# YunjiKim/Unsupervised-Keypoint-Learning-for-Guiding-Class-conditional-Video-Prediction

Measured on AMD Instinct MI355X. Metric: detector_translator train frames/sec @128x128 K=15, higher is better.
Workload: dtype f32

## Files before the change

unsupervised-keypoint-learning-for-guiding-class-conditional-video-prediction_amd/csrc/conv_wgrad.hip:

```cpp
#include "kpx_internal.h"
#include "kpx_bf16.h"
#include <cassert>

#ifdef __HIP_DEVICE_COMPILE__
__device__ __attribute__((aligned(16))) float kpx_zero16[4] = {0.f, 0.f, 0.f, 0.f};
#else
extern __device__ float kpx_zero16[4];
#endif


template <int BMc, int BNk, int WM, int WN, bool VEC, bool MERGE>
__global__ __launch_bounds__(WM * WN * 64) void conv_wgrad_kernel(const WgradGeom g) {
    constexpr int NT = WM * WN * 64;
    constexpr int BKP = 32;
    constexpr int TM = BMc / (WM * 32), TN = BNk / (WN * 32);
    constexpr int RA = (BKP * BMc / 4) / NT, RB = (BKP * BNk / 4) / NT;
    static_assert(RA >= 1 && RB >= 1 && TM >= 1 && TN >= 1, "tile/wave shape");
    __shared__ __attribute__((aligned(16))) float As[2][BKP * BMc];
    __shared__ __attribute__((aligned(16))) float Bs[2][BKP * BNk];

    const int t = threadIdx.x, lane = t & 63, wave = t >> 6;
    const int li = lane & 31, lh = lane >> 5;
    const int wm = wave / WN, wn = wave % WN;
    int L = kpx_xcd_remap(blockIdx.x, gridDim.x);
// ... 511 lines not shown
            const float* p = g.x + ((ptrdiff_t)(n * g.Hi + ih) * g.Wi + iw0) * g.Cin + xf[i];
            const float v = *(ok ? p : g.x);
            rx[i] = ok ? v : 0.f;
        }
        {
            const int k4 = t % (CoutT / 4), px = t / (CoutT / 4), k = k4 * 4;
            my = 0;
            if (k < g.Cout) { const int rem = g.Cout - k; my = rem >= 4 ? 15u : (15u >> (4 - rem)); }
            const float* p = g.dy + ((size_t)(n * g.Ho + ho) * g.Wo + wc * CW + px) * g.lddy + k;
            ry = *reinterpret_cast<const f32x4*>(my ? p : g.dy);
        }
    };
    auto store_chunk = [&](int buf) {
#pragma unroll
        for (int i = 0; i < RX; ++i) xs[buf][t + 256 * i] = rx[i];
        f32x4 o;
#pragma unroll
        for (int j = 0; j < 4; ++j) o[j] = (my >> j) & 1u ? ry[j] : 0.f;
        *reinterpret_cast<f32x4*>(&dys[buf][t * 4]) = o;
    };
    const int nch = cend > cbeg ? cend - cbeg : 0;
    if (nch > 0) { load_chunk(cbeg); store_chunk(0); }
    __syncthreads();
    for (int ch = 0; ch < nch; ++ch) {
        const int buf = ch & 1;
        const bool more = ch + 1 < nch;
        if (more) load_chunk(cbeg + ch + 1);
#pragma unroll
        for (int sl = 0; sl < 2; ++sl) {
            const int r = wave + 4 * sl;
            if (r < g.KH) {
                const float* Xr = &xs[buf][r * SEG];
#pragma unroll
                for (int s2 = 0; s2 < CW / 2; ++s2) {
                    const int kp = 2 * s2 + lh;
                    acc[sl] = __builtin_amdgcn_mfma_f32_32x32x2f32(Xr[kp * g.Cin + li], dys[buf][kp * CoutT + li], acc[sl], 0, 0, 0);
                }
            }
        }
        if (more) store_chunk(buf ^ 1);
        __syncthreads();
    }
    float* out = g.out + (size_t)split * g.slab;
#pragma unroll
    for (int sl = 0; sl < 2; ++sl) {
        const int r = wave + 4 * sl;
        if (r < g.KH) {
#pragma unroll
            for (int e = 0; e < 16; ++e) {
                const int c = (e & 3) + 8 * (e >> 2) + 4 * lh;
                if (c < KWC && li < g.Cout) out[((size_t)r * KWC + c) * g.Cout + li] = acc[sl][e];
            }
        }
    }
}

static bool wgrad_rows_merged_plan(int N, int Ho, int Wo, int Cin, int Cout, int KH, int KW, int* S, int* cpb) {
    if (Cin % 4 == 0 || KW * Cin > 32 || (32 + KW - 1) * Cin > 128 || KH > 8 || KW < 2 || Wo % 32 != 0 || Cout > 32 ||
        (long)N * Ho * Wo < 65536)
        return false;
    const long total = (long)N * Ho * (Wo / 32);
    long s = total < 768 ? total : 768;
    *cpb = (int)((total + s - 1) / s);
    *S = (int)((total + *cpb - 1) / *cpb);
    return true;
}

static bool wgrad_rows_plan(int N, int Ho, int Wo, int Cin, int Cout, int KH, int KW, int* S, int* cpb, int* CT) {
    if (KH > 3 || KW > 3 || KH * KW < 2 || Wo % 32 != 0 || Cout > 32 || Cin > 128 || (long)N * Ho * Wo < 65536) return false;
    *CT = Cin > 32 ? 2 : 1;
    const int ct = (Cin + 32 * *CT - 1) / (32 * *CT);
    const long total = (long)N * Ho * (Wo / 32);
    long want = 768 / ct;
    if (want < 1) want = 1;
    long s = total < want ? total : want;
    const size_t slab_bytes = (size_t)KH * KW * Cin * Cout * 4;
    const size_t cap = (size_t)256 << 20;
    if ((size_t)s * slab_bytes > cap) s = (long)(cap / slab_bytes);
    if (s < 1) s = 1;
    *cpb = (int)((total + s - 1) / s);
    *S = (int)((total + *cpb - 1) / *cpb);
    return true;
}

static void wgrad_tiles(int Cin, int Cout, int& bm, int& bn) {
    auto pick = [](int c) { return ((c + 127) / 128 * 128 == (c + 63) / 64 * 64) ? 128 : 64; };
    bm = pick(Cin); bn = pick(Cout);
    if (bm != bn) { bm = 64; bn = 64; }
}

static inline bool wgrad_merge(int Cin, int ldx, int KW) { return Cin % 4 != 0 && ldx == Cin && KW > 1 && KW * Cin <= 64; }

static int wgrad_splits(int N, int Ho, int Wo, int Cin, int Cout, int KH, int KW) {
    int bm, bn;
    wgrad_tiles(Cin, Cout, bm, bn);
    long tiles = (long)KH * KW * ((Cin + bm - 1) / bm) * ((Cout + bn - 1) / bn);
    if (wgrad_merge(Cin, Cin, KW)) tiles = (long)KH * ((Cout + bn - 1) / bn);
    const long P = (long)N * Ho * Wo;
    const long target = bm == 128 ? 2560 : 4096;
    long S = target / tiles;
    const long maxS_pix = P / 512 > 0 ? P / 512 : 1;
    if (S > maxS_pix) S = maxS_pix;
    const size_t slab_bytes = (size_t)KH * KW * Cin * Cout * 4;
    const size_t cap = (size_t)256 << 20;
    if ((size_t)S * slab_bytes > cap) S = (long)(cap / slab_bytes);
    if (S < 1) S = 1;
    return (int)S;
}

enum { WG_F32, WG_BF16, WG_IMAGE16 };
struct WgradCall : WgradGeom { int arith, types; };

struct WgradPlan {
    int family = -1;
    int S; size_t need;
    int cpb, CT, bm;
    WgradGeom g;
};

static bool wgrad_args_ok(const WgradCall& c) {
    if (!c.x || !c.dy || c.N <= 0 || c.Hi <= 0 || c.Wi <= 0 || c.Cin <= 0 || c.Cout <= 0 || c.Ho <= 0 || c.Wo <= 0 || c.KH <= 0 || c.KW <= 0 ||
        c.stride <= 0 || c.ldx < c.Cin || c.lddy < c.Cout || c.arith < 0 || c.arith > 1)
        return false;
    if (c.types == WG_BF16) return c.ldx % 8 == 0 && c.lddy % 8 == 0 && kpx_aligned16(c.x, c.dy);
    return c.types != WG_IMAGE16 || c.Cin <= 4;
}

template <class G>
static G wgrad_fill(const WgradPlan& p) {
    const WgradGeom& c = p.g;
    G g{};
    g.x = c.x; g.dy = c.dy; g.out = c.out;
    g.N = c.N; g.Hi = c.Hi; g.Wi = c.Wi; g.Cin = c.Cin; g.ldx = c.ldx;
    g.Ho = c.Ho; g.Wo = c.Wo; g.Cout = c.Cout; g.lddy = c.lddy;
    g.KH = c.KH; g.KW = c.KW; g.pad_t = c.pad_t; g.pad_l = c.pad_l;
    g.total_chunks = c.N * c.Ho * (c.Wo / 32); g.cpb = p.cpb; g.ct = c.ct; g.slab = c.slab;
    return g;
}

static WgradPlan wgrad_plan(const WgradCall& c) {
    WgradPlan p{};
    WgradGeom& g = p.g = c;
    g.slab = (size_t)c.KH * c.KW * c.Cin * c.Cout;
    const bool any = !c.x;
    auto take = [&](int family, int S) {
        p.family = family; p.S = S;
        if (S > 1 && (size_t)S * g.slab * 4 > p.need) p.need = (size_t)S * g.slab * 4;
        return !any;
    };
    g.vecA = any || (c.ldx % 4 == 0 && kpx_aligned16(c.x)); g.vecB = any || (c.lddy % 4 == 0 && kpx_aligned16(c.dy));
    const bool vec = g.vecA && g.vecB;
    const size_t px_in = (size_t)c.N * c.Hi * c.Wi, px_out = (size_t)c.N * c.Ho * c.Wo;
    int S, bn;

    if (c.types != WG_BF16 && kpx_offsets_fit(px_in, c.ldx, 0x60000000ull) && kpx_offsets_fit(px_out, c.lddy, 0x60000000ull) &&
        (any || (c.Cout % 4 == 0 && g.vecB)) && (c.Cin % 4 != 0 || g.vecA)) {
        S = kpx_wsmall_splits(c.N, c.Hi, c.Wi, c.Cin, c.Ho, c.Wo, c.Cout, c.KH, c.KW, c.stride);
        if (S >= 1 && take(KPX_WGRAD_WSMALL, S)) return p;
    }
    if (c.types == WG_IMAGE16) return p;
    if (c.types == WG_F32 && c.stride == 1) {
        if (c.KH == 3 && c.KW == 3 && c.pad_t == 1 && c.pad_l == 1 && c.Ho == c.Hi && c.Wo == c.Wi && vec && (any || c.ldx >= ((c.Cin + 3) & ~3)) &&
            kpx_offsets_fit(px_in, c.ldx > c.lddy ? c.ldx : c.lddy, 0x60000000ull)) {
            S = kpx_wino_wgrad_splits(c.N, c.Hi, c.Wi, c.Cin, c.Cout);
            if (S >= 1 && take(KPX_WGRAD_WINO, S)) return p;
        }
        g.ct = 1;
        if (c.ldx == c.Cin && g.vecB && wgrad_rows_merged_plan(c.N, c.Ho, c.Wo, c.Cin, c.Cout, c.KH, c.KW, &S, &p.cpb) && take(KPX_WGRAD_ROWS_MERGED, S))
            return p;
        if (vec && c.Cin % 4 == 0 && wgrad_rows_plan(c.N, c.Ho, c.Wo, c.Cin, c.Cout, c.KH, c.KW, &S, &p.cpb, &p.CT)) {
            g.ct = (c.Cin + 32 * p.CT - 1) / (32 * p.CT);
            if (take(KPX_WGRAD_ROWS, S)) return p;
        }
    }
    wgrad_tiles(c.Cin, c.Cout, p.bm, bn);
    g.ct = (c.Cin + p.bm - 1) / p.bm; g.kt = (c.Cout + bn - 1) / bn; g.P = (int)px_out;
    g.S = S = wgrad_splits(c.N, c.Ho, c.Wo, c.Cin, c.Cout, c.KH, c.KW);
    g.pps = ((g.P + S - 1) / S + 31) / 32 * 32;
    g.io16 = c.types == WG_BF16;
    g.terms = g.io16 || c.arith == KPX_ARITH_BF16 ? 1 : 3;
    const bool tap = c.types == WG_F32 && vec && c.Cin % 4 == 0 && c.Cout % 4 == 0 && c.Wo % 32 == 0;
    if (kpx_wgrad3_eligible(&g) && (c.stride > 1 || !tap) && take(KPX_WGRAD_GEMM3, S)) return p;
    if (c.types == WG_BF16) return p;
    if (tap) {
        const int chunks = c.N * c.Ho * (c.Wo / 32);
        p.cpb = (chunks + S - 1) / S;
        const int St = (chunks + p.cpb - 1) / p.cpb;
        assert(St <= S);
        if (take(KPX_WGRAD_TAP_ROWS, St)) return p;
    }
    if (wgrad_merge(c.Cin, c.ldx, c.KW)) {
        g.merge = c.Cin; g.Cin = c.KW * c.Cin; g.KW = 1; g.vecA = 0;
        g.ct = (g.Cin + p.bm - 1) / p.bm;
    }
    take(KPX_WGRAD_GENERIC, S);
    return p;
}

static int wgrad_run(const WgradCall& c, float* dw, void* workspace, size_t workspace_bytes, void* stream) {
    if (!dw || !wgrad_args_ok(c)) return KPX_EINVAL;
    WgradPlan p = wgrad_plan(c);
    if (p.family < 0 || p.need > (workspace ? workspace_bytes : 0)) return KPX_EINVAL;
    float* const out = p.g.out = p.S > 1 ? (float*)workspace : dw;
    hipStream_t s = kpx_stream(stream);
    int rc = 0;
    switch (p.family) {
        case KPX_WGRAD_WSMALL:
            rc = kpx_wsmall_launch(c.x, c.N, c.Hi, c.Wi, c.Cin, c.ldx, c.dy, c.Ho, c.Wo, c.Cout, c.lddy, c.KH, c.KW, c.stride, c.pad_t, c.pad_l, out, p.S, s,
                                   c.types == WG_IMAGE16);
            break;
        case KPX_WGRAD_WINO:
            rc = kpx_wino_wgrad3x3(c.x, c.N, c.Hi, c.Wi, c.Cin, c.ldx, c.dy, c.Cout, c.lddy, out, p.S, s);
            break;
        case KPX_WGRAD_ROWS_MERGED:
        case KPX_WGRAD_ROWS: {
            const WgradRowsGeom r = wgrad_fill<WgradRowsGeom>(p);
            const dim3 grid((unsigned)(p.S * r.ct));
            if (p.family == KPX_WGRAD_ROWS_MERGED) hipLaunchKernelGGL((conv_wgrad_rows_merged_kernel<0>), grid, dim3(256), 0, s, r);
            else if (p.CT == 2) hipLaunchKernelGGL((conv_wgrad_rows_kernel<2>), grid, dim3(256), 0, s, r);
            else hipLaunchKernelGGL((conv_wgrad_rows_kernel<1>), grid, dim3(256), 0, s, r);
            break;
        }
        case KPX_WGRAD_TAP_ROWS: {
            WgradTapGeom r = wgrad_fill<WgradTapGeom>(p);
            r.stride = c.stride; r.S = p.S; r.kt = p.g.kt;
            const dim3 grid((unsigned)(r.S * r.KH * r.KW * r.ct * r.kt));
            if (p.bm == 128) hipLaunchKernelGGL((conv_wgrad_tap_rows_kernel<128, 128, 2, 4>), grid, dim3(512), 0, s, r);
            else hipLaunchKernelGGL((conv_wgrad_tap_rows_kernel<64, 64, 2, 2>), grid, dim3(256), 0, s, r);
            break;
        }
        default: {
            const WgradGeom& g = p.g;
            const dim3 grid((unsigned)(g.S * g.KH * g.KW * g.ct * g.kt));
            const bool vec = g.vecA && g.vecB;
            if (p.family == KPX_WGRAD_GEMM3) rc = kpx_wgrad3_launch(g, p.bm, g.terms, s);
            else if (g.merge) hipLaunchKernelGGL((conv_wgrad_kernel<64, 64, 2, 2, false, true>), grid, dim3(256), 0, s, g);
            else if (p.bm == 128 && vec) hipLaunchKernelGGL((conv_wgrad_kernel<128, 128, 2, 4, true, false>), grid, dim3(512), 0, s, g);
            else if (p.bm == 128) hipLaunchKernelGGL((conv_wgrad_kernel<128, 128, 2, 4, false, false>), grid, dim3(512), 0, s, g);
            else if (vec) hipLaunchKernelGGL((conv_wgrad_kernel<64, 64, 2, 2, true, false>), grid, dim3(256), 0, s, g);
            else hipLaunchKernelGGL((conv_wgrad_kernel<64, 64, 2, 2, false, false>), grid, dim3(256), 0, s, g);
        }
    }
    return finish_wgrad(rc ? rc : kpx_launch_status(), workspace, dw, p.g.slab, p.S, s);
}

extern "C" int kpx_conv2d_wgrad_f32(const float* x, int N, int Hi, int Wi, int Cin, int ldx,
                                    const float* dy, int Ho, int Wo, int Cout, int lddy,
                                    float* dw, int KH, int KW, int stride, int pad_t, int pad_l, int arith,
                                    void* workspace, size_t workspace_bytes, void* stream) {
    return wgrad_run({{x, dy, nullptr, N, Hi, Wi, Cin, ldx, Ho, Wo, Cout, lddy, KH, KW, stride, pad_t, pad_l}, arith, WG_F32}, dw, workspace, workspace_bytes, stream);
}

extern "C" int kpx_conv2d_wgrad_bf16(const void* x, int N, int Hi, int Wi, int Cin, int ldx, const void* dy, int Ho, int Wo, int Cout, int lddy,
                                     float* dw, int KH, int KW, int stride, int pad_t, int pad_l, void* workspace, size_t workspace_bytes, void* stream) {
    return wgrad_run({{(const float*)x, (const float*)dy, nullptr, N, Hi, Wi, Cin, ldx, Ho, Wo, Cout, lddy, KH, KW, stride, pad_t, pad_l}, 0, WG_BF16},
                     dw, workspace, workspace_bytes, stream);
}

extern "C" int kpx_conv_image_wgrad_bf16(const float* x, int N, int Hi, int Wi, int Cin, int ldx, const void* dy, int Ho, int Wo, int Cout, int lddy,
                                         float* dw, int KH, int KW, int stride, int pad_t, int pad_l, void* workspace, size_t workspace_bytes, void* stream) {
    return wgrad_run({{x, (const float*)dy, nullptr, N, Hi, Wi, Cin, ldx, Ho, Wo, Cout, lddy, KH, KW, stride, pad_t, pad_l}, 0, WG_IMAGE16},
                     dw, workspace, workspace_bytes, stream);
}

extern "C" int kpx_conv2d_wgrad_plan(const float* x, int N, int Hi, int Wi, int Cin, int ldx, const float* dy, int Ho, int Wo, int Cout, int lddy,
                                     int KH, int KW, int stride, int pad_t, int pad_l, int arith, int* family, int* splits, size_t* workspace_bytes) {
    const WgradCall c{{x, dy, nullptr, N, Hi, Wi, Cin, ldx, Ho, Wo, Cout, lddy, KH, KW, stride, pad_t, pad_l}, arith, WG_F32};
    if (!family || !splits || !workspace_bytes || !wgrad_args_ok(c)) return KPX_EINVAL;
    const WgradPlan p = wgrad_plan(c);
    *family = p.family; *splits = p.S; *workspace_bytes = p.need;
    return 0;
}

extern "C" size_t kpx_conv2d_wgrad_workspace_bytes(int N, int Ho, int Wo, int Cin, int Cout, int KH, int KW) {
    auto need = [&](int st) { return wgrad_plan({{nullptr, nullptr, nullptr, N, Ho * st, Wo * st, Cin, Cin, Ho, Wo, Cout, Cout, KH, KW, st, 1, 1}, 0, WG_F32}).need; };
    return std::max(need(1), need(2));
}
```

unsupervised-keypoint-learning-for-guiding-class-conditional-video-prediction_amd/csrc/conv_wino.hip:

```cpp
#include "kpx_internal.h"
#include "kpx_env.h"
#include <stdlib.h>
#include <type_traits>
#include <atomic>

struct WinoGeom {
    const float* x; float* y; const float* U; const float* bias;
    int N, H, W, Cin, ldx, Cout, ldy, act;
    int pack;
    int Kp, Np;
    int tiles_y, tiles_x, nt;
    int stagger;
    float* stats;
    const float* mask_y; int ld_mask;
    const float* bn_beta;
};

static __device__ __attribute__((aligned(16))) float wino_zero16[4] = {0.f, 0.f, 0.f, 0.f};

template <bool DGRAD>
__global__ __launch_bounds__(256) void wino_filter_transform_frag_kernel(const float* __restrict__ w, int Cin, int Cout, int Kp, int Np, float* __restrict__ Uf) {
    const int K = DGRAD ? Cout : Cin, Nn = DGRAD ? Cin : Cout;
    const int KC = Kp >> 3, NB = Np >> 5;
    const size_t total = (size_t)Kp * Np;
// ... 296 lines not shown
    }
    if (STATS != 0) {
        __syncthreads();
        float* const S = smem;
        *reinterpret_cast<f32x4*>(&S[t * 8]) = st_s;
        *reinterpret_cast<f32x4*>(&S[t * 8 + 4]) = st_q;
        __syncthreads();
        if (t < 2 * NC) {
            const int stat = t / NC, c = t - stat * NC, cq = c >> 2, e = c & 3;
            float r = 0.f;
#pragma unroll 8
            for (int m = 0; m < 512 / (NC / 4); ++m) r += S[(cq + (NC / 4) * m) * 8 + stat * 4 + e];
            const size_t tile_id = ((size_t)n * g.tiles_y + by) * g.tiles_x + bx;
            if (n0 + c < g.Cout) g.stats[(tile_id * 2 + stat) * g.Cout + n0 + c] = r;
        }
    }
#ifdef KPX_WINO_STAMP
    if (dbg) { dbg[3] = __builtin_amdgcn_s_memtime(); dbg[4] = __builtin_amdgcn_s_memrealtime(); }
#endif
}

static inline int w2_lds_bytes(int mode) { const int main = W2_MAIN * 4, epi = 4 * 2 * 64 * 32 * mode * 4; return main > epi ? main : epi; }

static std::atomic<unsigned long long> wino_attr_mask{0};

extern "C" int kpx_conv3x3_wino_eligible(int N, int H, int W, int K, int Nn, int ldin, const void* in_ptr) {
    if (kpx_env()->no_wino || N <= 0 || K <= 0 || Nn <= 0) return 0;
    const bool shape = (H % 16 == 0 && W % 16 == 0) || (H == 8 && W == 8 && N % 4 == 0);
    const int kmin = 4, nmin = 4;
    const bool kfit = ldin >= ((K + 7) & ~7) || K == 4;
    return shape && K >= kmin && Nn >= nmin && (K >= 16 || K == 4 || K == 8) && kfit && (ldin % 4 == 0) && (((uintptr_t)in_ptr) & 15) == 0;
}
extern "C" __attribute__((visibility("hidden"))) int kpx_wino_eligible(int N, int H, int W, int K, int Nn, int ldin, const void* in_ptr) {
    return kpx_conv3x3_wino_eligible(N, H, W, K, Nn, ldin, in_ptr);
}

extern "C" size_t kpx_wino_u_bytes(int Cin, int Cout) {
    const size_t a = (size_t)((Cin + 7) & ~7) * ((Cout + 31) & ~31), b = (size_t)((Cout + 7) & ~7) * ((Cin + 31) & ~31);
    return 16 * 4 * (a > b ? a : b);
}

extern "C" int kpx_wino_filter_transform_f32(const float* w_hwio, int Cin, int Cout, int dgrad, float* U, void* stream) {
    if (!w_hwio || !U || Cin <= 0 || Cout <= 0) return KPX_EINVAL;
    const int K = dgrad ? Cout : Cin, Nn = dgrad ? Cin : Cout;
    const int Kp = (K + 7) & ~7, Np = (Nn + 31) & ~31;
    const size_t pairs = (size_t)Kp * Np;
    size_t nb = (pairs + 255) / 256; if (nb > 1024) nb = 1024;
    hipStream_t s = kpx_stream(stream);
    if (dgrad) hipLaunchKernelGGL(wino_filter_transform_frag_kernel<true>, dim3((unsigned)nb), dim3(256), 0, s, w_hwio, Cin, Cout, Kp, Np, U);
    else hipLaunchKernelGGL(wino_filter_transform_frag_kernel<false>, dim3((unsigned)nb), dim3(256), 0, s, w_hwio, Cin, Cout, Kp, Np, U);
    return kpx_launch_status();
}

__global__ __launch_bounds__(256) void wino_filter_transform_batch_kernel(const KpxWinoDesc* __restrict__ descs) {
    const KpxWinoDesc d = descs[blockIdx.y];
    const int Cin = d.cin, Cout = d.cout;
    const bool dg = d.dgrad != 0;
    const int K = dg ? Cout : Cin, Nn = dg ? Cin : Cout;
    const int Kp = (K + 7) & ~7, Np = (Nn + 31) & ~31, KC = Kp >> 3, NB = Np >> 5;
    const size_t total = (size_t)Kp * Np, pstride = (size_t)KC * NB * 256;
    const float* __restrict__ w = d.w;
    float* __restrict__ Uf = d.u;
    for (size_t idx = (size_t)blockIdx.x * 256 + threadIdx.x; idx < total; idx += (size_t)gridDim.x * 256) {
        const int j = (int)(idx & 3), li = (int)((idx >> 2) & 31), lh = (int)((idx >> 7) & 1);
        const size_t blk = idx >> 8;
        const int nb = (int)(blk % NB), kc = (int)(blk / NB);
        const int c = 8 * kc + 4 * lh + j, n = 32 * nb + li;
        const bool real = c < K && n < Nn;
        float g[3][3];
#pragma unroll
        for (int r = 0; r < 3; ++r)
#pragma unroll
            for (int q = 0; q < 3; ++q)
                g[r][q] = !real ? 0.f : (dg ? w[((size_t)((2 - r) * 3 + (2 - q)) * Cin + n) * Cout + c] : w[((size_t)(r * 3 + q) * Cin + c) * Cout + n]);
        float t[4][3];
#pragma unroll
        for (int q = 0; q < 3; ++q) {
            t[0][q] = g[0][q];
            t[1][q] = 0.5f * (g[0][q] + g[1][q] + g[2][q]);
            t[2][q] = 0.5f * (g[0][q] - g[1][q] + g[2][q]);
            t[3][q] = g[2][q];
        }
        float* o = Uf + blk * 256 + (idx & 255);
#pragma unroll
        for (int i = 0; i < 4; ++i) {
            o[(size_t)(i * 4 + 0) * pstride] = t[i][0];
            o[(size_t)(i * 4 + 1) * pstride] = 0.5f * (t[i][0] + t[i][1] + t[i][2]);
            o[(size_t)(i * 4 + 2) * pstride] = 0.5f * (t[i][0] - t[i][1] + t[i][2]);
            o[(size_t)(i * 4 + 3) * pstride] = t[i][2];
        }
    }
}
extern "C" int kpx_wino_filter_transform_batch_f32(const void* descs_dev, int n, void* stream) {
    if (!descs_dev || n <= 0 || n > 65535) return KPX_EINVAL;
    hipLaunchKernelGGL(wino_filter_transform_batch_kernel, dim3(64, (unsigned)n), dim3(256), 0, kpx_stream(stream), (const KpxWinoDesc*)descs_dev);
    return kpx_launch_status();
}

extern "C" size_t kpx_conv3x3_wino_stats_tiles(int N, int H, int W) {
    return (H % 16 || W % 16 || N <= 0) ? 0 : (size_t)N * (H / 16) * (W / 16);
}
static int wino_launch(const float* in, int N, int H, int W, int K, int ldin, const float* U, const float* bias,
                       float* out, int Nn, int ldout, int act, float* tile_stats, void* stream,
                       const float* mask_y, int ld_mask, const float* bn_beta) {
    if (!in || !U || !out || ldin < (K == 4 ? 4 : K) || ldout < Nn || act < 0 || act > 2 || !kpx_conv3x3_wino_eligible(N, H, W, K, Nn, ldin, in)) return KPX_EINVAL;
    hipStream_t s = kpx_stream(stream);
    if (kpx_first_use_on_device(&wino_attr_mask)) {
        hipError_t e = hipSuccess;
#define W2_ATTR(M, S) if (e == hipSuccess) e = hipFuncSetAttribute(reinterpret_cast<const void*>(conv_wino_v2_kernel<M, S>), hipFuncAttributeMaxDynamicSharedMemorySize, w2_lds_bytes(M))
        W2_ATTR(1, 0); W2_ATTR(2, 0); W2_ATTR(1, 1); W2_ATTR(2, 1); W2_ATTR(1, 2); W2_ATTR(2, 2);
#undef W2_ATTR
        if (e != hipSuccess) return -(int)e;
    }
    WinoGeom g{};
    g.x = in; g.y = out; g.U = U; g.bias = bias; g.stats = tile_stats;
    g.mask_y = mask_y; g.ld_mask = ld_mask; g.bn_beta = bn_beta;
    g.N = N; g.H = H; g.W = W; g.Cin = K; g.ldx = ldin; g.Cout = Nn; g.ldy = ldout; g.act = act;
    g.Kp = (K + 7) & ~7; g.Np = (Nn + 31) & ~31;
    g.pack = (H == 8 && W == 8) ? 1 : 0;
    g.tiles_y = g.pack ? 1 : H / 16; g.tiles_x = g.pack ? 1 : W / 16; g.nt = g.Np / 32;
    const unsigned blocks = (unsigned)((size_t)(g.pack ? N / 4 : N) * g.tiles_y * g.tiles_x * g.nt);
    const bool wide = blocks / 2 >= 256 && g.Np % 64 == 0;
    g.stagger = 1;
    const int st = !tile_stats ? 0 : (mask_y ? 2 : 1);
#define W2_GO(M, S) hipLaunchKernelGGL((conv_wino_v2_kernel<M, S>), dim3(M == 2 ? blocks / 2 : blocks), dim3(512), w2_lds_bytes(M), s, g)
    if (wide) { if (st == 0) W2_GO(2, 0); else if (st == 1) W2_GO(2, 1); else W2_GO(2, 2); }
    else { if (st == 0) W2_GO(1, 0); else if (st == 1) W2_GO(1, 1); else W2_GO(1, 2); }
#undef W2_GO
    return kpx_launch_status();
}

extern "C" int kpx_conv3x3_wino_f32(const float* in, int N, int H, int W, int K, int ldin, const float* U, const float* bias,
                                    float* out, int Nn, int ldout, int act, float* tile_stats, const float* bn_y, int ld_bn_y,
                                    const float* bn_beta, void* stream) {
    if (tile_stats && (H % 16 || W % 16)) return KPX_EINVAL;
    if ((bn_y || bn_beta) && (!tile_stats || !bn_y || !bn_beta || ld_bn_y < Nn || bias || act != KPX_ACT_NONE)) return KPX_EINVAL;
    return wino_launch(in, N, H, W, K, ldin, U, bias, out, Nn, ldout, act, tile_stats, stream, bn_y, ld_bn_y, bn_beta);
}

extern "C" __attribute__((visibility("hidden"))) int kpx_wino_conv3x3(const float* in, int N, int H, int W, int K, int ldin, const float* w_hwio, int Cin, int Cout, int dgrad,
                                const float* bias, int act, float* out, int Nn, int ldout, float* U_ws, hipStream_t s) {
    int rc = kpx_wino_filter_transform_f32(w_hwio, Cin, Cout, dgrad, U_ws, (void*)s);
    if (rc) return rc;
    return kpx_conv3x3_wino_f32(in, N, H, W, K, ldin, U_ws, bias, out, Nn, ldout, act, nullptr, nullptr, 0, nullptr, (void*)s);
}

struct WinoWgradGeom {
    const float* x; const float* dy; float* out;
    int N, H, W, Cin, ldx, Cout, lddy;
    int cit, cot, S, cps, total_chunks, chy, chx;
    size_t slab;
};

template <int CIT, int COT>
__global__ __launch_bounds__(512, 2) void conv_wino_wgrad_kernel(const WinoWgradGeom g) {
    constexpr int CI = 32 * CIT, CO = 32 * COT, SI = CI / 4, SO = CO / 4;
    constexpr int VF = 16 * 8 * CI, DF = 16 * 8 * CO, BUF = VF + DF;
    extern __shared__ __attribute__((aligned(16))) float smem[];

    const int t = threadIdx.x, lane = t & 63, wave = __builtin_amdgcn_readfirstlane(t >> 6), li = lane & 31, lh = lane >> 5;
    int L = kpx_xcd_remap(blockIdx.x, gridDim.x);
    const int split = L % g.S; L /= g.S;
    const int cot = L % g.cot, cit = L / g.cot;
    const int c0 = cit * CI, n0 = cot * CO;

    const int vsl = (t % SI) * 4, vtile = (t / SI) & 7, vrow = t / (8 * SI);
    const int esl = (t % SO) * 4, etile = (t / SO) & 7, erow = t / (8 * SO);
    const bool vthr = t < 32 * SI, ethr = t < 32 * SO;
    const bool vact = vthr && c0 + vsl < g.Cin, eact = ethr && n0 + esl < g.Cout;
    const int xtail = g.Cin - (c0 + vsl);
    const int ra = vrow == 0 ? 0 : (vrow == 2 ? 2 : 1), rb = vrow == 0 ? 2 : (vrow == 1 ? 2 : (vrow == 2 ? 1 : 3));
    const float sgn = vrow == 1 ? 1.f : -1.f;
    const int pya = 2 * (vtile >> 2) + ra - 1, pyb = 2 * (vtile >> 2) + rb - 1, px0 = 2 * (vtile & 3) - 1;
    const int vwr = (vrow * 4) * 8 * CI + vtile * CI + vsl;
    const float d0 = erow == 3 ? 0.f : 1.f, d1 = erow == 0 ? 0.f : (erow == 1 ? 1.f : -1.f);
    const int dwr = VF + (erow * 4) * 8 * CO + etile * CO + esl;
    const int dyo = ((2 * (etile >> 2) * g.W + 2 * (etile & 3)) * g.lddy + n0 + esl) * 4;
    const int OOB = (int)0x80000000;
    const __amdgpu_buffer_rsrc_t rsx = __builtin_amdgcn_make_buffer_rsrc(const_cast<float*>(g.x) - (size_t)(g.W + 1) * g.ldx, 0, 0x7fffffff, 0x00020000);
    const __amdgpu_buffer_rsrc_t rsd = __builtin_amdgcn_make_buffer_rsrc(const_cast<float*>(g.dy), 0, 0x7fffffff, 0x00020000);
    int vxa[4], vxb[4], vd[4];
#pragma unroll
    for (int c = 0; c < 4; ++c) {
        vxa[c] = vact ? (((pya + 1) * g.W + px0 + c + 1) * g.ldx + c0 + vsl) * 4 : OOB;
        vxb[c] = vact ? (((pyb + 1) * g.W + px0 + c + 1) * g.ldx + c0 + vsl) * 4 : OOB;
    }
    vd[0] = eact ? dyo : OOB; vd[1] = eact ? dyo + g.lddy * 4 : OOB; vd[2] = eact ? dyo + g.W * g.lddy * 4 : OOB; vd[3] = eact ? dyo + (g.W + 1) * g.lddy * 4 : OOB;
    const bool top_a = pya < 0, bot_a = pya > 3, top_b = pyb < 0, bot_b = pyb > 3, left0 = px0 < 0, right3 = px0 + 3 > 7;
    const int p0 = 2 * wave;

    f32x16 acc[2][CIT][COT];
#pragma unroll
    for (int a = 0; a < 2; ++a)
#pragma unroll
        for (int b = 0; b < CIT; ++b)
#pragma unroll
            for (int c = 0; c < COT; ++c)
#pragma unroll
                for (int r = 0; r < 16; ++r) acc[a][b][c][r] = 0.f;

    const int ch_begin = split * g.cps;
    int ch_end = ch_begin + g.cps; if (ch_end > g.total_chunks) ch_end = g.total_chunks;
    const int nch = ch_end - ch_begin;
    const int lq = ch_begin / g.chx;
    int lcx = __builtin_amdgcn_readfirstlane(ch_begin - lq * g.chx);
    int lcy = __builtin_amdgcn_readfirstlane(lq % g.chy), ln = __builtin_amdgcn_readfirstlane(lq / g.chy);
    f32x4 rxa[4], rxb[4], rd[4];
    auto load_next = [&]() {
        const int pix = (ln * g.H + lcy * 4) * g.W + lcx * 8;
        const int sx = pix * g.ldx * 4, sd = pix * g.lddy * 4;
        const bool s_top = lcy == 0, s_bot = lcy + 1 == g.chy, s_left = lcx == 0, s_right = lcx + 1 == g.chx;
        const bool inv_a = (top_a && s_top) || (bot_a && s_bot), inv_b = (top_b && s_top) || (bot_b && s_bot);
#pragma unroll
        for (int c = 0; c < 4; ++c) {
            const bool inv_c = (c == 0 && left0 && s_left) || (c == 3 && right3 && s_right);
            rxa[c] = __builtin_bit_cast(f32x4, __builtin_amdgcn_raw_buffer_load_b128(rsx, (inv_a || inv_c) ? OOB : vxa[c], sx, 0));
            rxb[c] = __builtin_bit_cast(f32x4, __builtin_amdgcn_raw_buffer_load_b128(rsx, (inv_b || inv_c) ? OOB : vxb[c], sx, 0));
        }
#pragma unroll
        for (int i = 0; i < 4; ++i) rd[i] = __builtin_bit_cast(f32x4, __builtin_amdgcn_raw_buffer_load_b128(rsd, vd[i], sd, 0));
        if (++lcx == g.chx) { lcx = 0; if (++lcy == g.chy) { lcy = 0; ++ln; } }
    };
    auto transform = [&](float* buf) {
        if (vthr) {
            f32x4 tr[4];
#pragma unroll
            for (int c = 0; c < 4; ++c) tr[c] = rxa[c] + sgn * rxb[c];
            if (g.Cin & 3) {
#pragma unroll
                for (int c = 0; c < 4; ++c)
#pragma unroll
                    for (int j = 1; j < 4; ++j) if (j >= xtail) tr[c][j] = 0.f;
            }
            *reinterpret_cast<f32x4*>(&buf[vwr]) = tr[0] - tr[2];
            *reinterpret_cast<f32x4*>(&buf[vwr + 8 * CI]) = tr[1] + tr[2];
            *reinterpret_cast<f32x4*>(&buf[vwr + 16 * CI]) = tr[2] - tr[1];
            *reinterpret_cast<f32x4*>(&buf[vwr + 24 * CI]) = tr[1] - tr[3];
        }
        if (ethr) {
            const f32x4 t0 = d0 * rd[0] + d1 * rd[2], t1 = d0 * rd[1] + d1 * rd[3];
            *reinterpret_cast<f32x4*>(&buf[dwr]) = t0;
            *reinterpret_cast<f32x4*>(&buf[dwr + 8 * CO]) = t0 + t1;
            *reinterpret_cast<f32x4*>(&buf[dwr + 16 * CO]) = t0 - t1;
            *reinterpret_cast<f32x4*>(&buf[dwr + 24 * CO]) = -t1;
        }
    };
    auto mfma = [&](const float* buf) {
#pragma unroll
        for (int pt = 0; pt < 2; ++pt) {
            const float* Vp = buf + (p0 + pt) * 8 * CI + lh * CI + li;
            const float* Dp = buf + VF + (p0 + pt) * 8 * CO + lh * CO + li;
#pragma unroll
            for (int s = 0; s < 4; ++s) {
                float a[CIT], b[COT];
#pragma unroll
                for (int i = 0; i < CIT; ++i) a[i] = Vp[s * 2 * CI + i * 32];
#pragma unroll
                for (int j = 0; j < COT; ++j) b[j] = Dp[s * 2 * CO + j * 32];
#pragma unroll
                for (int i = 0; i < CIT; ++i)
#pragma unroll
                    for (int j = 0; j < COT; ++j)
                        acc[pt][i][j] = __builtin_amdgcn_mfma_f32_32x32x2f32(a[i], b[j], acc[pt][i][j], 0, 0, 0);
            }
        }
    };
    const bool late = wave >= 4;
    if (nch > 0) {
        load_next();
        transform(smem);
        if (nch > 1) load_next();
    }
    for (int k = 0; k < nch; ++k) {
        float* const cur = smem + (k & 1) * BUF;
        float* const nxt = smem + ((k & 1) ^ 1) * BUF;
        __syncthreads();
        if (late) mfma(cur);
        if (k + 1 < nch) transform(nxt);
        if (k + 2 < nch) load_next();
        if (!late) mfma(cur);
    }
    __syncthreads();

    float* Ms = smem;
    float* out = g.out + (size_t)split * g.slab;
    const int oc = t & 31;
#pragma unroll
    for (int q = 0; q < CIT * COT; ++q) {
        const int ci = q / COT, co = q % COT;
        if (q) __syncthreads();
#pragma unroll
        for (int pt = 0; pt < 2; ++pt)
#pragma unroll
            for (int r = 0; r < 16; ++r)
                Ms[((p0 + pt) * 32 + (r & 3) + 8 * (r >> 2) + 4 * lh) * 32 + li] = acc[pt][ci][co][r];
        __syncthreads();
#pragma unroll
        for (int i = 0; i < 2; ++i) {
            const int cl = (t >> 5) + 16 * i;
            float m[16];
#pragma unroll
            for (int p = 0; p < 16; ++p) m[p] = Ms[(p * 32 + cl) * 32 + oc];
            float h[3][4];
#pragma unroll
            for (int j = 0; j < 4; ++j) {
                h[0][j] = m[j] + 0.5f * (m[4 + j] + m[8 + j]);
                h[1][j] = 0.5f * (m[4 + j] - m[8 + j]);
                h[2][j] = 0.5f * (m[4 + j] + m[8 + j]) + m[12 + j];
            }
            const int c = c0 + ci * 32 + cl, n = n0 + co * 32 + oc;
            if (c < g.Cin && n < g.Cout) {
                float* o = out + (size_t)c * g.Cout + n;
                const size_t tap = (size_t)g.Cin * g.Cout;
#pragma unroll
                for (int r = 0; r < 3; ++r) {
                    o[(r * 3 + 0) * tap] = h[r][0] + 0.5f * (h[r][1] + h[r][2]);
                    o[(r * 3 + 1) * tap] = 0.5f * (h[r][1] - h[r][2]);
                    o[(r * 3 + 2) * tap] = 0.5f * (h[r][1] + h[r][2]) + h[r][3];
                }
            }
        }
    }
}

static inline int ww_tile(int C) { return (C % 64 == 0 || C > 96) ? 2 : 1; }

extern "C" __attribute__((visibility("hidden"))) int kpx_wino_wgrad_splits(int N, int H, int W, int Cin, int Cout) {
    if (kpx_env()->no_wino) return 0;
    const int comin = 4;
    if (H % 4 || W % 8 || Cout % 4 || Cin < 32 || Cout < comin) return 0;
    const int ti = ww_tile(Cin), to = ww_tile(Cout);
    if (ti == 1 && to == 1) return 0;
    const long tc = (long)N * (H / 4) * (W / 8), tiles = (long)((Cin + 32 * ti - 1) / (32 * ti)) * ((Cout + 32 * to - 1) / (32 * to));
    const long target = 256;
    long S = target / tiles;
    if (S < 1) S = 1;
    if (S > tc / 8) S = tc / 8;
    const long cap = (128L << 20) / ((long)9 * Cin * Cout * 4);
    if (S > cap) S = cap;
    if (S < 1) S = 1;
    if (tc < 64 || tiles * S < 128) return 0;
    return (int)S;
}

extern "C" __attribute__((visibility("hidden"))) int kpx_wino_wgrad3x3(const float* x, int N, int H, int W, int Cin, int ldx, const float* dy, int Cout, int lddy,
                                                                   float* slabs, int S, hipStream_t s) {
    static std::atomic<unsigned long long> attr_mask{0};
    const int lds22 = 2 * (16 * 8 * 64 + 16 * 8 * 64) * 4, lds21 = 2 * (16 * 8 * 64 + 16 * 8 * 32) * 4, lds12 = 2 * (16 * 8 * 32 + 16 * 8 * 64) * 4;
    if (kpx_first_use_on_device(&attr_mask)) {
        hipError_t e = hipFuncSetAttribute(reinterpret_cast<const void*>(conv_wino_wgrad_kernel<2, 2>), hipFuncAttributeMaxDynamicSharedMemorySize, lds22);
        if (e == hipSuccess) e = hipFuncSetAttribute(reinterpret_cast<const void*>(conv_wino_wgrad_kernel<2, 1>), hipFuncAttributeMaxDynamicSharedMemorySize, lds21 > 65536 ? lds21 : 65536);
        if (e == hipSuccess) e = hipFuncSetAttribute(reinterpret_cast<const void*>(conv_wino_wgrad_kernel<1, 2>), hipFuncAttributeMaxDynamicSharedMemorySize, lds12 > 65536 ? lds12 : 65536);
        if (e != hipSuccess) return -(int)e;
    }
    const int ti = ww_tile(Cin), to = ww_tile(Cout);
    WinoWgradGeom g{};
    g.x = x; g.dy = dy; g.out = slabs;
    g.N = N; g.H = H; g.W = W; g.Cin = Cin; g.ldx = ldx; g.Cout = Cout; g.lddy = lddy;
    g.cit = (Cin + 32 * ti - 1) / (32 * ti); g.cot = (Cout + 32 * to - 1) / (32 * to); g.S = S;
    g.chy = H / 4; g.chx = W / 8; g.total_chunks = N * g.chy * g.chx;
    g.cps = (g.total_chunks + S - 1) / S;
    g.slab = (size_t)9 * Cin * Cout;
    const dim3 grid((unsigned)(g.cit * g.cot * S));
    if (ti == 2 && to == 2) hipLaunchKernelGGL((conv_wino_wgrad_kernel<2, 2>), grid, dim3(512), lds22, s, g);
    else if (ti == 2) hipLaunchKernelGGL((conv_wino_wgrad_kernel<2, 1>), grid, dim3(512), lds21 > 65536 ? lds21 : 65536, s, g);
    else hipLaunchKernelGGL((conv_wino_wgrad_kernel<1, 2>), grid, dim3(512), lds12 > 65536 ? lds12 : 65536, s, g);
    return kpx_launch_status();
}
```

unsupervised-keypoint-learning-for-guiding-class-conditional-video-prediction_amd/csrc/kpx_env.h:

```cpp
#pragma once

struct KpxEnv {
    int no_wino;
    int no_gemm3;
    int bf16s_variant;
};

extern "C" __attribute__((visibility("hidden"))) const KpxEnv* kpx_env();
```

unsupervised-keypoint-learning-for-guiding-class-conditional-video-prediction_amd/csrc/kpx_env.hip:

```cpp
#include <stdio.h>
#include <stdlib.h>
#include <atomic>
#include <mutex>
#include "kpx_env.h"
#include "../../include/kpx.h"

static KpxEnv g_env;
static std::atomic<int> g_env_loaded{0};
static std::mutex g_env_mutex;

static int env_flag(const char* name) { return getenv(name) != nullptr; }
static long env_long(const char* name, long dflt) { const char* v = getenv(name); return v ? atol(v) : dflt; }

static void env_parse(KpxEnv* e) {
    e->no_wino = env_flag("KPX_NO_WINO");
    e->no_gemm3 = env_flag("KPX_NO_GEMM3");
    e->bf16s_variant = (int)env_long("KPX_BF16S_VARIANT", 0);
}

extern "C" __attribute__((visibility("hidden"))) const KpxEnv* kpx_env() {
    if (!g_env_loaded.load(std::memory_order_acquire)) {
        std::lock_guard<std::mutex> lock(g_env_mutex);
        if (!g_env_loaded.load(std::memory_order_relaxed)) {
            env_parse(&g_env);
            g_env_loaded.store(1, std::memory_order_release);
        }
    }
    return &g_env;
}

extern "C" int kpx_reload_env(void) {
    std::lock_guard<std::mutex> lock(g_env_mutex);
    env_parse(&g_env);
    g_env_loaded.store(1, std::memory_order_release);
    return 0;
}
```

unsupervised-keypoint-learning-for-guiding-class-conditional-video-prediction_amd/csrc/kpx_internal.h:

```cpp
#pragma once
#include "conv_geom.h"

static inline bool kpx_offsets_fit(size_t pixels, size_t ld, size_t limit) { return pixels * ld * 4 < limit; }

extern "C" __attribute__((visibility("hidden"))) int kpx_gemm3_eligible(const ConvGeom* g);
extern "C" __attribute__((visibility("hidden"))) int kpx_gemm3_launch(ConvGeom g, int bt, int terms, hipStream_t s);
extern "C" __attribute__((visibility("hidden"))) int kpx_wgrad3_eligible(const WgradGeom* g);
extern "C" __attribute__((visibility("hidden"))) int kpx_wgrad3_launch(WgradGeom g, int bm, int terms, hipStream_t s);

extern "C" __attribute__((visibility("hidden"))) int kpx_wino_eligible(int N, int H, int W, int K, int Nn, int ldin, const void* in_ptr);
extern "C" __attribute__((visibility("hidden"))) int kpx_wino_conv3x3(const float* in, int N, int H, int W, int K, int ldin, const float* w_hwio, int Cin, int Cout, int dgrad,
                                const float* bias, int act, float* out, int Nn, int ldout, float* U_ws, hipStream_t s);
extern "C" __attribute__((visibility("hidden"))) int kpx_wino_wgrad_splits(int N, int H, int W, int Cin, int Cout);
extern "C" __attribute__((visibility("hidden"))) int kpx_wino_wgrad3x3(const float* x, int N, int H, int W, int Cin, int ldx, const float* dy, int Cout, int lddy,
                                 float* slabs, int S, hipStream_t s);

extern "C" __attribute__((visibility("hidden"))) int kpx_conv_rgb_fwd(const float* x, int N, int Hi, int Wi, int Cin, const float* w, int KH, int KW,
                                const float* bias, float* y, int Ho, int Wo, int Cout, int ldy,
                                int stride, int pad_t, int pad_l, int act, hipStream_t s, int y16 = 0);
extern "C" __attribute__((visibility("hidden"))) int kpx_conv_rgb_dgrad(const float* dy, int N, int Ho, int Wo, int Cout, int lddy, const float* w, int KH, int KW,
                                  float* dx, int Hi, int Wi, int Cin, int lddx, int stride, int pad_t, int pad_l, hipStream_t s, int dy16 = 0);
extern "C" __attribute__((visibility("hidden"))) int kpx_conv_few_fwd(const float* x, int N, int Hi, int Wi, int Cin, int ldx, const float* w, int KH, int KW,
                                const float* bias, float* y, int Ho, int Wo, int Cout, int ldy,
                                int stride, int pad_t, int pad_l, int act, hipStream_t s);

extern "C" __attribute__((visibility("hidden"))) int kpx_wsmall_splits(int N, int Hi, int Wi, int Cin, int Ho, int Wo, int Cout, int KH, int KW, int stride);
extern "C" __attribute__((visibility("hidden"))) int kpx_wsmall_launch(const float* x, int N, int Hi, int Wi, int Cin, int ldx, const float* dy, int Ho, int Wo, int Cout, int lddy,
                                 int KH, int KW, int stride, int pad_t, int pad_l, float* slabs, int S, hipStream_t s, int dy16 = 0);
```

Before: 1424.

## Route thin-channel 3x3 weight gradients through Winograd with 16-tile chunks

Adds a Winograd weight-gradient variant for layers where both Cin and Cout fit a single 32-wide tile. The kernel is templated on tiles per chunk and instantiated with 16 tiles (8-row chunks), so each block does more MFMA work per load. The planner tries this path before the small-weight kernel, and an env flag that defaults to on controls it. This cuts wgrad arithmetic for thin convolutions. It costs larger LDS use and possibly less parallelism per chunk, and it takes over layers that previously went to the wsmall kernel.

```diff
diff --git a/unsupervised-keypoint-learning-for-guiding-class-conditional-video-prediction_amd/csrc/conv_wgrad.hip b/unsupervised-keypoint-learning-for-guiding-class-conditional-video-prediction_amd/csrc/conv_wgrad.hip
--- a/unsupervised-keypoint-learning-for-guiding-class-conditional-video-prediction_amd/csrc/conv_wgrad.hip
+++ b/unsupervised-keypoint-learning-for-guiding-class-conditional-video-prediction_amd/csrc/conv_wgrad.hip
@@ -687,6 +687,12 @@
     const bool vec = g.vecA && g.vecB;
     const size_t px_in = (size_t)c.N * c.Hi * c.Wi, px_out = (size_t)c.N * c.Ho * c.Wo;
     int S, bn;
+    const bool wino = c.types == WG_F32 && c.stride == 1 && c.KH == 3 && c.KW == 3 && c.pad_t == 1 && c.pad_l == 1 && c.Ho == c.Hi && c.Wo == c.Wi && vec &&
+                      (any || c.ldx >= ((c.Cin + 3) & ~3)) && kpx_offsets_fit(px_in, c.ldx > c.lddy ? c.ldx : c.lddy, 0x60000000ull);
+    if (wino && kpx_wino_wgrad_thin(c.Cin, c.Cout)) {
+        S = kpx_wino_wgrad_splits(c.N, c.Hi, c.Wi, c.Cin, c.Cout);
+        if (S >= 1 && take(KPX_WGRAD_WINO, S)) return p;
+    }
 
     if (c.types != WG_BF16 && kpx_offsets_fit(px_in, c.ldx, 0x60000000ull) && kpx_offsets_fit(px_out, c.lddy, 0x60000000ull) &&
         (any || (c.Cout % 4 == 0 && g.vecB)) && (c.Cin % 4 != 0 || g.vecA)) {
@@ -695,8 +701,7 @@
     }
     if (c.types == WG_IMAGE16) return p;
     if (c.types == WG_F32 && c.stride == 1) {
-        if (c.KH == 3 && c.KW == 3 && c.pad_t == 1 && c.pad_l == 1 && c.Ho == c.Hi && c.Wo == c.Wi && vec && (any || c.ldx >= ((c.Cin + 3) & ~3)) &&
-            kpx_offsets_fit(px_in, c.ldx > c.lddy ? c.ldx : c.lddy, 0x60000000ull)) {
+        if (wino && !kpx_wino_wgrad_thin(c.Cin, c.Cout)) {
             S = kpx_wino_wgrad_splits(c.N, c.Hi, c.Wi, c.Cin, c.Cout);
             if (S >= 1 && take(KPX_WGRAD_WINO, S)) return p;
         }
diff --git a/unsupervised-keypoint-learning-for-guiding-class-conditional-video-prediction_amd/csrc/conv_wino.hip b/unsupervised-keypoint-learning-for-guiding-class-conditional-video-prediction_amd/csrc/conv_wino.hip
--- a/unsupervised-keypoint-learning-for-guiding-class-conditional-video-prediction_amd/csrc/conv_wino.hip
+++ b/unsupervised-keypoint-learning-for-guiding-class-conditional-video-prediction_amd/csrc/conv_wino.hip
@@ -472,10 +472,11 @@
     size_t slab;
 };
 
-template <int CIT, int COT>
+template <int CIT, int COT, int TPC = 8>
 __global__ __launch_bounds__(512, 2) void conv_wino_wgrad_kernel(const WinoWgradGeom g) {
     constexpr int CI = 32 * CIT, CO = 32 * COT, SI = CI / 4, SO = CO / 4;
-    constexpr int VF = 16 * 8 * CI, DF = 16 * 8 * CO, BUF = VF + DF;
+    constexpr int PR = TPC / 2;
+    constexpr int VF = 16 * TPC * CI, DF = 16 * TPC * CO, BUF = VF + DF;
     extern __shared__ __attribute__((aligned(16))) float smem[];
 
     const int t = threadIdx.x, lane = t & 63, wave = __builtin_amdgcn_readfirstlane(t >> 6), li = lane & 31, lh = lane >> 5;
@@ -484,17 +485,17 @@
     const int cot = L % g.cot, cit = L / g.cot;
     const int c0 = cit * CI, n0 = cot * CO;
 
-    const int vsl = (t % SI) * 4, vtile = (t / SI) & 7, vrow = t / (8 * SI);
-    const int esl = (t % SO) * 4, etile = (t / SO) & 7, erow = t / (8 * SO);
-    const bool vthr = t < 32 * SI, ethr = t < 32 * SO;
+    const int vsl = (t % SI) * 4, vtile = (t / SI) & (TPC - 1), vrow = t / (TPC * SI);
+    const int esl = (t % SO) * 4, etile = (t / SO) & (TPC - 1), erow = t / (TPC * SO);
+    const bool vthr = t < 4 * TPC * SI, ethr = t < 4 * TPC * SO;
     const bool vact = vthr && c0 + vsl < g.Cin, eact = ethr && n0 + esl < g.Cout;
     const int xtail = g.Cin - (c0 + vsl);
     const int ra = vrow == 0 ? 0 : (vrow == 2 ? 2 : 1), rb = vrow == 0 ? 2 : (vrow == 1 ? 2 : (vrow == 2 ? 1 : 3));
     const float sgn = vrow == 1 ? 1.f : -1.f;
     const int pya = 2 * (vtile >> 2) + ra - 1, pyb = 2 * (vtile >> 2) + rb - 1, px0 = 2 * (vtile & 3) - 1;
-    const int vwr = (vrow * 4) * 8 * CI + vtile * CI + vsl;
+    const int vwr = (vrow * 4) * TPC * CI + vtile * CI + vsl;
     const float d0 = erow == 3 ? 0.f : 1.f, d1 = erow == 0 ? 0.f : (erow == 1 ? 1.f : -1.f);
-    const int dwr = VF + (erow * 4) * 8 * CO + etile * CO + esl;
+    const int dwr = VF + (erow * 4) * TPC * CO + etile * CO + esl;
     const int dyo = ((2 * (etile >> 2) * g.W + 2 * (etile & 3)) * g.lddy + n0 + esl) * 4;
     const int OOB = (int)0x80000000;
     const __amdgpu_buffer_rsrc_t rsx = __builtin_amdgcn_make_buffer_rsrc(const_cast<float*>(g.x) - (size_t)(g.W + 1) * g.ldx, 0, 0x7fffffff, 0x00020000);
@@ -506,7 +507,7 @@
         vxb[c] = vact ? (((pyb + 1) * g.W + px0 + c + 1) * g.ldx + c0 + vsl) * 4 : OOB;
     }
     vd[0] = eact ? dyo : OOB; vd[1] = eact ? dyo + g.lddy * 4 : OOB; vd[2] = eact ? dyo + g.W * g.lddy * 4 : OOB; vd[3] = eact ? dyo + (g.W + 1) * g.lddy * 4 : OOB;
-    const bool top_a = pya < 0, bot_a = pya > 3, top_b = pyb < 0, bot_b = pyb > 3, left0 = px0 < 0, right3 = px0 + 3 > 7;
+    const bool top_a = pya < 0, bot_a = pya > PR - 1, top_b = pyb < 0, bot_b = pyb > PR - 1, left0 = px0 < 0, right3 = px0 + 3 > 7;
     const int p0 = 2 * wave;
 
     f32x16 acc[2][CIT][COT];
@@ -527,7 +528,7 @@
     int lcy = __builtin_amdgcn_readfirstlane(lq % g.chy), ln = __builtin_amdgcn_readfirstlane(lq / g.chy);
     f32x4 rxa[4], rxb[4], rd[4];
     auto load_next = [&]() {
-        const int pix = (ln * g.H + lcy * 4) * g.W + lcx * 8;
+        const int pix = (ln * g.H + lcy * PR) * g.W + lcx * 8;
         const int sx = pix * g.ldx * 4, sd = pix * g.lddy * 4;
         const bool s_top = lcy == 0, s_bot = lcy + 1 == g.chy, s_left = lcx == 0, s_right = lcx + 1 == g.chx;
         const bool inv_a = (top_a && s_top) || (bot_a && s_bot), inv_b = (top_b && s_top) || (bot_b && s_bot);
@@ -553,25 +554,25 @@
                     for (int j = 1; j < 4; ++j) if (j >= xtail) tr[c][j] = 0.f;
             }
             *reinterpret_cast<f32x4*>(&buf[vwr]) = tr[0] - tr[2];
-            *reinterpret_cast<f32x4*>(&buf[vwr + 8 * CI]) = tr[1] + tr[2];
-            *reinterpret_cast<f32x4*>(&buf[vwr + 16 * CI]) = tr[2] - tr[1];
-            *reinterpret_cast<f32x4*>(&buf[vwr + 24 * CI]) = tr[1] - tr[3];
+            *reinterpret_cast<f32x4*>(&buf[vwr + TPC * CI]) = tr[1] + tr[2];
+            *reinterpret_cast<f32x4*>(&buf[vwr + 2 * TPC * CI]) = tr[2] - tr[1];
+            *reinterpret_cast<f32x4*>(&buf[vwr + 3 * TPC * CI]) = tr[1] - tr[3];
         }
         if (ethr) {
             const f32x4 t0 = d0 * rd[0] + d1 * rd[2], t1 = d0 * rd[1] + d1 * rd[3];
             *reinterpret_cast<f32x4*>(&buf[dwr]) = t0;
-            *reinterpret_cast<f32x4*>(&buf[dwr + 8 * CO]) = t0 + t1;
-            *reinterpret_cast<f32x4*>(&buf[dwr + 16 * CO]) = t0 - t1;
-            *reinterpret_cast<f32x4*>(&buf[dwr + 24 * CO]) = -t1;
+            *reinterpret_cast<f32x4*>(&buf[dwr + TPC * CO]) = t0 + t1;
+            *reinterpret_cast<f32x4*>(&buf[dwr + 2 * TPC * CO]) = t0 - t1;
+            *reinterpret_cast<f32x4*>(&buf[dwr + 3 * TPC * CO]) = -t1;
         }
     };
     auto mfma = [&](const float* buf) {
 #pragma unroll
         for (int pt = 0; pt < 2; ++pt) {
-            const float* Vp = buf + (p0 + pt) * 8 * CI + lh * CI + li;
-            const float* Dp = buf + VF + (p0 + pt) * 8 * CO + lh * CO + li;
-#pragma unroll
-            for (int s = 0; s < 4; ++s) {
+            const float* Vp = buf + (p0 + pt) * TPC * CI + lh * CI + li;
+            const float* Dp = buf + VF + (p0 + pt) * TPC * CO + lh * CO + li;
+#pragma unroll
+            for (int s = 0; s < TPC / 2; ++s) {
                 float a[CIT], b[COT];
 #pragma unroll
                 for (int i = 0; i < CIT; ++i) a[i] = Vp[s * 2 * CI + i * 32];
@@ -645,13 +646,16 @@
 
 static inline int ww_tile(int C) { return (C % 64 == 0 || C > 96) ? 2 : 1; }
 
+extern "C" __attribute__((visibility("hidden"))) int kpx_wino_wgrad_thin(int Cin, int Cout) { return ww_tile(Cin) == 1 && ww_tile(Cout) == 1; }
+
 extern "C" __attribute__((visibility("hidden"))) int kpx_wino_wgrad_splits(int N, int H, int W, int Cin, int Cout) {
     if (kpx_env()->no_wino) return 0;
     const int comin = 4;
     if (H % 4 || W % 8 || Cout % 4 || Cin < 32 || Cout < comin) return 0;
     const int ti = ww_tile(Cin), to = ww_tile(Cout);
-    if (ti == 1 && to == 1) return 0;
-    const long tc = (long)N * (H / 4) * (W / 8), tiles = (long)((Cin + 32 * ti - 1) / (32 * ti)) * ((Cout + 32 * to - 1) / (32 * to));
+    const bool thin = ti == 1 && to == 1;
+    if (thin && (!kpx_env()->wino_wgrad_thin || H % 8 || Cout < 32)) return 0;
+    const long tc = (long)N * (H / (thin ? 8 : 4)) * (W / 8), tiles = (long)((Cin + 32 * ti - 1) / (32 * ti)) * ((Cout + 32 * to - 1) / (32 * to));
     const long target = 256;
     long S = target / tiles;
     if (S < 1) S = 1;
@@ -667,10 +671,12 @@
                                                                    float* slabs, int S, hipStream_t s) {
     static std::atomic<unsigned long long> attr_mask{0};
     const int lds22 = 2 * (16 * 8 * 64 + 16 * 8 * 64) * 4, lds21 = 2 * (16 * 8 * 64 + 16 * 8 * 32) * 4, lds12 = 2 * (16 * 8 * 32 + 16 * 8 * 64) * 4;
+    const int lds11 = 2 * (16 * 16 * 32 + 16 * 16 * 32) * 4;
     if (kpx_first_use_on_device(&attr_mask)) {
         hipError_t e = hipFuncSetAttribute(reinterpret_cast<const void*>(conv_wino_wgrad_kernel<2, 2>), hipFuncAttributeMaxDynamicSharedMemorySize, lds22);
         if (e == hipSuccess) e = hipFuncSetAttribute(reinterpret_cast<const void*>(conv_wino_wgrad_kernel<2, 1>), hipFuncAttributeMaxDynamicSharedMemorySize, lds21 > 65536 ? lds21 : 65536);
         if (e == hipSuccess) e = hipFuncSetAttribute(reinterpret_cast<const void*>(conv_wino_wgrad_kernel<1, 2>), hipFuncAttributeMaxDynamicSharedMemorySize, lds12 > 65536 ? lds12 : 65536);
+        if (e == hipSuccess) e = hipFuncSetAttribute(reinterpret_cast<const void*>(conv_wino_wgrad_kernel<1, 1, 16>), hipFuncAttributeMaxDynamicSharedMemorySize, lds11);
         if (e != hipSuccess) return -(int)e;
     }
     const int ti = ww_tile(Cin), to = ww_tile(Cout);
@@ -678,12 +684,15 @@
     g.x = x; g.dy = dy; g.out = slabs;
     g.N = N; g.H = H; g.W = W; g.Cin = Cin; g.ldx = ldx; g.Cout = Cout; g.lddy = lddy;
     g.cit = (Cin + 32 * ti - 1) / (32 * ti); g.cot = (Cout + 32 * to - 1) / (32 * to); g.S = S;
-    g.chy = H / 4; g.chx = W / 8; g.total_chunks = N * g.chy * g.chx;
+    const bool thin = ti == 1 && to == 1;
+    if (thin && H % 8) return KPX_EINVAL;
+    g.chy = H / (thin ? 8 : 4); g.chx = W / 8; g.total_chunks = N * g.chy * g.chx;
     g.cps = (g.total_chunks + S - 1) / S;
     g.slab = (size_t)9 * Cin * Cout;
     const dim3 grid((unsigned)(g.cit * g.cot * S));
     if (ti == 2 && to == 2) hipLaunchKernelGGL((conv_wino_wgrad_kernel<2, 2>), grid, dim3(512), lds22, s, g);
     else if (ti == 2) hipLaunchKernelGGL((conv_wino_wgrad_kernel<2, 1>), grid, dim3(512), lds21 > 65536 ? lds21 : 65536, s, g);
-    else hipLaunchKernelGGL((conv_wino_wgrad_kernel<1, 2>), grid, dim3(512), lds12 > 65536 ? lds12 : 65536, s, g);
+    else if (to == 2) hipLaunchKernelGGL((conv_wino_wgrad_kernel<1, 2>), grid, dim3(512), lds12 > 65536 ? lds12 : 65536, s, g);
+    else hipLaunchKernelGGL((conv_wino_wgrad_kernel<1, 1, 16>), grid, dim3(512), lds11, s, g);
     return kpx_launch_status();
 }
diff --git a/unsupervised-keypoint-learning-for-guiding-class-conditional-video-prediction_amd/csrc/kpx_env.h b/unsupervised-keypoint-learning-for-guiding-class-conditional-video-prediction_amd/csrc/kpx_env.h
--- a/unsupervised-keypoint-learning-for-guiding-class-conditional-video-prediction_amd/csrc/kpx_env.h
+++ b/unsupervised-keypoint-learning-for-guiding-class-conditional-video-prediction_amd/csrc/kpx_env.h
@@ -3,6 +3,7 @@
 struct KpxEnv {
     int no_wino;
     int no_gemm3;
+    int wino_wgrad_thin;
     int bf16s_variant;
 };
 
diff --git a/unsupervised-keypoint-learning-for-guiding-class-conditional-video-prediction_amd/csrc/kpx_env.hip b/unsupervised-keypoint-learning-for-guiding-class-conditional-video-prediction_amd/csrc/kpx_env.hip
--- a/unsupervised-keypoint-learning-for-guiding-class-conditional-video-prediction_amd/csrc/kpx_env.hip
+++ b/unsupervised-keypoint-learning-for-guiding-class-conditional-video-prediction_amd/csrc/kpx_env.hip
@@ -15,6 +15,7 @@
 static void env_parse(KpxEnv* e) {
     e->no_wino = env_flag("KPX_NO_WINO");
     e->no_gemm3 = env_flag("KPX_NO_GEMM3");
+    e->wino_wgrad_thin = env_long("KPX_WINO_WGRAD_THIN", 1) != 0;
     e->bf16s_variant = (int)env_long("KPX_BF16S_VARIANT", 0);
 }
 
diff --git a/unsupervised-keypoint-learning-for-guiding-class-conditional-video-prediction_amd/csrc/kpx_internal.h b/unsupervised-keypoint-learning-for-guiding-class-conditional-video-prediction_amd/csrc/kpx_internal.h
--- a/unsupervised-keypoint-learning-for-guiding-class-conditional-video-prediction_amd/csrc/kpx_internal.h
+++ b/unsupervised-keypoint-learning-for-guiding-class-conditional-video-prediction_amd/csrc/kpx_internal.h
@@ -12,6 +12,7 @@
 extern "C" __attribute__((visibility("hidden"))) int kpx_wino_conv3x3(const float* in, int N, int H, int W, int K, int ldin, const float* w_hwio, int Cin, int Cout, int dgrad,
                                 const float* bias, int act, float* out, int Nn, int ldout, float* U_ws, hipStream_t s);
 extern "C" __attribute__((visibility("hidden"))) int kpx_wino_wgrad_splits(int N, int H, int W, int Cin, int Cout);
+extern "C" __attribute__((visibility("hidden"))) int kpx_wino_wgrad_thin(int Cin, int Cout);
 extern "C" __attribute__((visibility("hidden"))) int kpx_wino_wgrad3x3(const float* x, int N, int H, int W, int Cin, int ldx, const float* dy, int Cout, int lddy,
                                  float* slabs, int S, hipStream_t s);
 
```

New measurement: 1435, median of 6. About the same (+0.8%).
